# LLNL/Juqbox.jl

Hardware: AMD Instinct MI355X
Metric: traceobjgrad evals/sec (fwd+adjoint), cnot3 Hilbert dim (higher is better)
Workload: dtype f64

## Files before the change

### juqbox.jl_amd/csrc/jq_kernels.h

```cpp
#pragma once
#include <hip/hip_runtime.h>
#include <stdint.h>
#include <type_traits>

typedef double d4 __attribute__((ext_vector_type(4)));

#define JQ_WAVES 4
#define JQ_MAXNC 4
#define JQ_NTR 5
#define JQ_STATE_ARRAYS 4
#define JQ_STATE_EXTRA 8
#define JQ_MAXSLOTS 2
#define JQ_MAXSCHED 30

#define JQ_BW_OD 9
#define JQ_OD_COEFS(NT) (32 * (NT))

#define JQ_BW_T4 8
#define JQ_BW_T4Q 7
#define JQ_T4_AIDX(rho, k, i) (((rho) >> 2) * 64 + 16 * (k) + 4 * ((rho) & 3) + (i))
#define JQ_T4_TILE 16
#define JQ_T4_COEFS(NT) (64 * (NT))
#define JQ_T4_CIDX(g, r, t) ((g) * 16 + (r) * 4 + (t))
#define JQ_T4_CPOS(r, t) (4 * (r) + (t))
// ... 56 lines not shown
__device__ __forceinline__ s1 operator*(const s1& a, const s1& b) { return s1(a.e[0] * b.e[0]); }
__device__ __forceinline__ s1 operator*(double c, const s1& b) { return s1(c * b.e[0]); }
__device__ __forceinline__ s1 operator-(const s1& a) { return s1(-a.e[0]); }
__device__ __forceinline__ double row_sum(const d4& p) { return (p[0] + p[1]) + (p[2] + p[3]); }
__device__ __forceinline__ double row_sum(const s4& p) { return (p[0] + p[1]) + (p[2] + p[3]); }
__device__ __forceinline__ double row_sum(const s1& p) { return p[0]; }
#if defined(JQ_BW) && JQ_BW == 7
typedef s1 jq_row;
#define JQ_RL 1
#elif defined(JQ_BW) && JQ_BW == 8 && !defined(JQ_ROW_D4)
typedef s4 jq_row;
#define JQ_RL 4
#else
typedef d4 jq_row;
#define JQ_RL 4
#endif

template <int NT>
struct Arr {
    jq_row t[NT];
};

template <int NT>
__device__ __forceinline__ void a_zero(Arr<NT>& a)
{
#pragma unroll
    for (int i = 0; i < NT; ++i) a.t[i] = (d4){0.0, 0.0, 0.0, 0.0};
}
template <int NT>
__device__ __forceinline__ void a_axpy(Arr<NT>& y, double c, const Arr<NT>& x)
{
#pragma unroll
    for (int i = 0; i < NT; ++i) y.t[i] += c * x.t[i];
}
template <int NT>
__device__ __forceinline__ void a_add(Arr<NT>& y, const Arr<NT>& x)
{
#pragma unroll
    for (int i = 0; i < NT; ++i) y.t[i] += x.t[i];
}
template <int NT>
__device__ __forceinline__ void a_neg(Arr<NT>& y)
{
#pragma unroll
    for (int i = 0; i < NT; ++i) y.t[i] = -y.t[i];
}
template <int NT>
__device__ __forceinline__ double a_dot(const Arr<NT>& x, const Arr<NT>& y)
{
    double s = 0.0;
#pragma unroll
    for (int i = 0; i < NT; ++i) {
#if JQ_RL == 1 && defined(JQ_EXP_DOTFMA)
        s = fma(x.t[i][0], y.t[i][0], s);
#else
        s += row_sum(x.t[i] * y.t[i]);
#endif
    }
    return s;
}
template <int NT>
__device__ __forceinline__ void a_axpy_rows(Arr<NT>& y, double c, const double* tab, int g, const Arr<NT>& x)
{
#if JQ_RL == 1
#pragma unroll
    for (int i = 0; i < NT; ++i) y.t[i][0] = fma(c * tab[16 * i + g], x.t[i][0], y.t[i][0]);
#else
    const d4* t4 = (const d4*)(tab + 4 * g);
#pragma unroll
    for (int i = 0; i < NT; ++i) y.t[i] += jq_row(c * t4[4 * i]) * x.t[i];
#endif
}
template <int NT, bool NEG>
__device__ __forceinline__ void a_axpy_rows1(Arr<NT>& y, const double* tab, int g, const Arr<NT>& x)
{
#if JQ_RL == 1
#pragma unroll
    for (int i = 0; i < NT; ++i) y.t[i][0] = fma(NEG ? -tab[16 * i + g] : tab[16 * i + g], x.t[i][0], y.t[i][0]);
#else
    const d4* t4 = (const d4*)(tab + 4 * g);
#pragma unroll
    for (int i = 0; i < NT; ++i) y.t[i] += jq_row(NEG ? -t4[4 * i] : t4[4 * i]) * x.t[i];
#endif
}
template <int NT>
__device__ __forceinline__ double a_wsq(const double* tab, int g, const Arr<NT>& x)
{
    double s = 0.0;
#pragma unroll
    for (int i = 0; i < NT; ++i)
#pragma unroll
        for (int r = 0; r < JQ_RL; ++r) s += tab[16 * i + (JQ_RL == 1 ? g : 4 * g + r)] * (x.t[i][r] * x.t[i][r]);
    return s;
}

template <int NT>
__device__ __forceinline__ void a_load(Arr<NT>& a, const double* __restrict__ img, int lane)
{
#pragma unroll
    for (int i = 0; i < NT; ++i)
#pragma unroll
        for (int r = 0; r < JQ_RL; ++r) a.t[i][r] = img[(4 * i + r) * 64 + lane];
}
template <int NT>
__device__ __forceinline__ void a_store(const Arr<NT>& a, double* __restrict__ img, int lane)
{
#pragma unroll
    for (int i = 0; i < NT; ++i)
#pragma unroll
        for (int r = 0; r < JQ_RL; ++r) img[(4 * i + r) * 64 + lane] = a.t[i][r];
}

#define JQ_PF 4

template <int NT, bool ZEROC, bool SD>
__device__ __forceinline__ void mm_od(Arr<NT>& D, const Arr<NT>& C, const double* mat, const Arr<NT>& x)
{
    constexpr int NTILES = SD ? 0 : 4 * NT;
    const int lane = threadIdx.x & 63;
    const double* cf = mat - lane + NTILES * 64 + (lane >> 4) * 4;
    const d4 zero = {0.0, 0.0, 0.0, 0.0};
    d4 ca = *(const d4*)(cf), cb = *(const d4*)(cf + 16);
    if constexpr (SD) {
        d4 x_prev = zero, x_cur = x.t[0];
#pragma unroll
        for (int mt = 0; mt < NT; ++mt) {
            const d4 x_next = (mt + 1 < NT) ? x.t[mt + 1] : zero;
            d4 acc = ZEROC ? zero : C.t[mt];
            if (mt > 0) acc += ca * x_prev;
            if (mt + 1 < NT) acc += cb * x_next;
            if (mt + 1 < NT) {
                ca = *(const d4*)(cf + ((mt + 1) * 2 + 0) * 16);
                cb = *(const d4*)(cf + ((mt + 1) * 2 + 1) * 16);
            }
            D.t[mt] = acc;
            x_prev = x_cur;
            x_cur = x_next;
        }
        return;
    } else {
        double f[JQ_PF];
#pragma unroll
        for (int i = 0; i < JQ_PF; ++i)
            if (i < NTILES) f[i] = mat[i * 64];
        d4 x_cur = x.t[0];
        d4 nxt = ZEROC ? zero : C.t[0];
        if (NT > 1) nxt += cb * x.t[1];
        if (NT > 1) {
            ca = *(const d4*)(cf + 2 * 16);
            cb = *(const d4*)(cf + 3 * 16);
        }
#pragma unroll
        for (int mt = 0; mt < NT; ++mt) {
            const d4 x_next = (mt + 1 < NT) ? x.t[mt + 1] : zero;
            d4 acc = nxt;
#pragma unroll
            for (int k = 0; k < 4; ++k) {
                const int kk = 4 * mt + k;
                const double a = f[kk % JQ_PF];
                if (kk + JQ_PF < NTILES) f[kk % JQ_PF] = mat[(kk + JQ_PF) * 64];
                acc = __builtin_amdgcn_mfma_f64_16x16x4f64(a, x_cur[k], acc, 0, 0, 0);
                __builtin_amdgcn_sched_barrier(0);
                if (k == 0 && mt + 1 < NT) {
                    nxt = ZEROC ? zero : C.t[mt + 1];
                    nxt += ca * x_cur;
                    if (mt + 2 < NT) nxt += cb * x.t[mt + 2];
// ... 286 lines not shown
};
template <int NT, int NP, bool Z0, bool Z1, bool Z2, int SH = 0, typename HOOK = T4qNoHook, int SCM = 0>
__device__ __forceinline__ void mm_t4q_multi(Arr<NT>& D0, const Arr<NT>& C0, const double* m0, Arr<NT>& D1, const Arr<NT>& C1,
                                             const double* m1, Arr<NT>& D2, const Arr<NT>& C2, const double* m2, const Arr<NT>& x,
                                             double sh0 = 0.0, double sh1 = 0.0, double sh2 = 0.0, const double* wsr = nullptr,
                                             HOOK hook = HOOK())
{
    const int lane = threadIdx.x & 63;
    const double* ma[3] = {t4q_a(m0, lane), t4q_a(m1, lane), t4q_a(NP > 2 ? m2 : m1, lane)};
    const d4* cf[3] = {t4q_c<NT>(m0, lane), t4q_c<NT>(m1, lane), t4q_c<NT>(NP > 2 ? m2 : m1, lane)};
    double xold = 0.0;
    double as[3];
    d2 cs[3];
#pragma unroll
    for (int k = 0; k < NP; ++k)
        if ((SCM >> k) & 1) {
            as[k] = ma[k][0];
            cs[k] = t4s_c01(cf[k]);
        }
#pragma unroll
    for (int mt = 0; mt < NT; ++mt) {
        double a[3];
        d4 c[3];
#pragma unroll
        for (int k = 0; k < NP; ++k) {
            if ((SCM >> k) & 1) {
                a[k] = as[k];
                c[k] = t4s_c(cs[k], t4s_c23(cf[k], mt));
            } else {
                a[k] = ma[k][mt * 64];
                c[k] = t4q_cload(cf[k], mt);
            }
        }
        if constexpr (SH != 0) {
            const double w = wsr[16 * mt];
            if constexpr (SH & 1) a[0] = fma(sh0, w, a[0]);
            if constexpr (NP > 1 && (SH & 2)) a[1] = fma(sh1, w, a[1]);
            if constexpr (NP > 2 && (SH & 4)) a[2] = fma(sh2, w, a[2]);
        }
        const double xc = x.t[mt][0], xn = x.t[mt + 1 < NT ? mt + 1 : mt][0];
        const double su = row_shift4<0x114>(xc), sd = row_shift4<0x104>(xc);
        hook(mt, su, sd);
        double acc[3] = {Z0 ? 0.0 : C0.t[mt][0], (NP > 1 && !Z1) ? C1.t[mt][0] : 0.0, (NP > 2 && !Z2) ? C2.t[mt][0] : 0.0};
#ifndef JQ_EXP_MFMA_LAST
#pragma unroll
        for (int k = 0; k < NP; ++k) acc[k] = __builtin_amdgcn_mfma_f64_4x4x4f64(a[k], xc, acc[k], 0, 0, 0);
#endif
#pragma unroll
        for (int k = 0; k < NP; ++k) acc[k] = fma(c[k][0], su, acc[k]);
#pragma unroll
        for (int k = 0; k < NP; ++k) acc[k] = fma(c[k][1], sd, acc[k]);
        if (mt > 0) {
#pragma unroll
            for (int k = 0; k < NP; ++k) acc[k] = fma(c[k][2], xold, acc[k]);
        }
        if (mt + 1 < NT) {
#pragma unroll
            for (int k = 0; k < NP; ++k) acc[k] = fma(c[k][3], xn, acc[k]);
        }
#ifdef JQ_EXP_MFMA_LAST
#pragma unroll
        for (int k = 0; k < NP; ++k) acc[k] = __builtin_amdgcn_mfma_f64_4x4x4f64(a[k], xc, acc[k], 0, 0, 0);
#endif
        xold = xc;
        D0.t[mt][0] = acc[0];
        if constexpr (NP > 1) D1.t[mt][0] = acc[1];
        if constexpr (NP > 2) D2.t[mt][0] = acc[2];
        __builtin_amdgcn_sched_barrier(0);
    }
}
template <int NT, bool Z0, bool Z1, int SH = 0, int SCM = 0>
__device__ __forceinline__ void mm_t4q2(Arr<NT>& D0, const Arr<NT>& C0, const double* m0, Arr<NT>& D1, const Arr<NT>& C1,
                                        const double* m1, const Arr<NT>& x, double sh0 = 0.0, double sh1 = 0.0, const double* wsr = nullptr)
{
    mm_t4q_multi<NT, 2, Z0, Z1, true, SH, T4qNoHook, SCM>(D0, C0, m0, D1, C1, m1, D1, C1, m1, x, sh0, sh1, 0.0, wsr);
}
template <int NT, bool Z0, bool Z1, bool Z2, int SH = 0, int SCM = 0>
__device__ __forceinline__ void mm_t4q3(Arr<NT>& D0, const Arr<NT>& C0, const double* m0, Arr<NT>& D1, const Arr<NT>& C1,
                                        const double* m1, Arr<NT>& D2, const Arr<NT>& C2, const double* m2, const Arr<NT>& x,
                                        double sh0 = 0.0, double sh1 = 0.0, double sh2 = 0.0, const double* wsr = nullptr)
{
    mm_t4q_multi<NT, 3, Z0, Z1, Z2, SH, T4qNoHook, SCM>(D0, C0, m0, D1, C1, m1, D2, C2, m2, x, sh0, sh1, sh2, wsr);
}
template <int NT>
__device__ __forceinline__ void t4q_load(OpQ<NT>& op, const double* mat)
{
    const int lane = threadIdx.x & 63;
    const double* ma = t4q_a(mat, lane);
    const d4* cf = t4q_c<NT>(mat, lane);
#pragma unroll
    for (int mt = 0; mt < NT; ++mt) {
        op.a[mt] = ma[mt * 64];
#ifdef JQ_EXP_OPQ_EDGE
        const double* cd = (const double*)(cf + mt * 16);
        op.c[mt][0] = cd[0], op.c[mt][1] = cd[1];
        op.c[mt][2] = mt > 0 ? cd[2] : 0.0;
        op.c[mt][3] = mt + 1 < NT ? cd[3] : 0.0;
#else
        op.c[mt] = t4q_cload(cf, mt);
#endif
    }
}
template <int NT>
__device__ __forceinline__ void mm_t4q_regs(Arr<NT>& D, const Arr<NT>& C, const OpQ<NT>& op, const Arr<NT>& x)
{
    double xold = 0.0;
#pragma unroll
    for (int mt = 0; mt < NT; ++mt) t4q_block<NT, false, JQ_T4_DIAG | JQ_T4_RTERMS | JQ_T4_MTERMS>(D, C, x, mt, op.a[mt], op.c[mt], xold);
}

template <int NT>
struct OpS {
    double a;
    d2 c;
    d2 m[NT];
};
template <int NT>
__device__ __forceinline__ void t4s_load(OpS<NT>& op, const double* mat)
{
    const int lane = threadIdx.x & 63;
    const d4* cf = t4q_c<NT>(mat, lane);
    op.a = t4q_a(mat, lane)[0];
    op.c = t4s_c01(cf);
#pragma unroll
    for (int mt = 0; mt < NT; ++mt) op.m[mt] = t4s_c23(cf, mt);
}
template <int NT>
__device__ __forceinline__ void mm_t4s_regs(Arr<NT>& D, const Arr<NT>& C, const OpS<NT>& op, const Arr<NT>& x)
{
    double xold = 0.0;
#pragma unroll
    for (int mt = 0; mt < NT; ++mt)
        t4q_block<NT, false, JQ_T4_DIAG | JQ_T4_RTERMS | JQ_T4_MTERMS>(D, C, x, mt, op.a, t4s_c(op.c, op.m[mt]), xold);
}
template <int NT, bool ZEROC>
__device__ __forceinline__ void mm_t4s(Arr<NT>& D, const Arr<NT>& C, const double* mat, const Arr<NT>& x)
{
    const int lane = threadIdx.x & 63;
    const d4* cf = t4q_c<NT>(mat, lane);
    const double a = t4q_a(mat, lane)[0];
    const d2 c01 = t4s_c01(cf);
    d2 m_cur = t4s_c23(cf, 0);
    double xold = 0.0;
#pragma unroll
    for (int mt = 0; mt < NT; ++mt) {
        const d2 m = m_cur;
        if (mt + 1 < NT) m_cur = t4s_c23(cf, mt + 1);
        t4q_block<NT, ZEROC, JQ_T4_DIAG | JQ_T4_RTERMS | JQ_T4_MTERMS>(D, C, x, mt, a, t4s_c(c01, m), xold);
    }
}

template <int NT, int BW, bool ZEROC, bool SD = false>
__device__ __forceinline__ void mm_band(Arr<NT>& D, const Arr<NT>& C, const double* mat, const Arr<NT>& x);
template <int NT, int BW, bool ZEROC, bool SD = false>
__device__ __forceinline__ void mm_any(Arr<NT>& D, const Arr<NT>& C, const double* mat, const Arr<NT>& x)
{
    if constexpr (BW == JQ_BW_T4)
        mm_t4<NT, ZEROC, JQ_T4_DIAG | JQ_T4_RTERMS | JQ_T4_MTERMS>(D, C, mat, x);
    else if constexpr (BW == JQ_BW_T4Q)
        mm_t4q<NT, ZEROC, JQ_T4_DIAG | JQ_T4_RTERMS | JQ_T4_MTERMS>(D, C, mat, x);
    else if constexpr (BW == JQ_BW_OD)
        mm_od<NT, ZEROC, SD>(D, C, mat, x);
    else
        mm_band<NT, BW, ZEROC, SD>(D, C, mat, x);
}
template <int NT, int BW, bool ZEROC, bool SD>
// ... 54 lines not shown
        case JQ_T4_MTERMS: mm_t4q<NT, true, JQ_T4_MTERMS>(D, D, mat, x); break;
        default: mm_t4q<NT, true, JQ_T4_DIAG | JQ_T4_RTERMS | JQ_T4_MTERMS>(D, D, mat, x); break;
        }
    } else {
        if (BW > 0 && mode == 0)
            mm_any<NT, 0, true>(D, D, mat, x);
        else if (BW > 0 && NT > 1 && mode == 2)
            mm_any<NT, BW, true, true>(D, D, mat, x);
        else
            mm_any<NT, BW, true>(D, D, mat, x);
    }
}

template <int N>
__device__ __forceinline__ double row_ror_add(double x)
{
    union {
        double d;
        int i[2];
    } a, b;
    a.d = x;
    b.i[0] = __builtin_amdgcn_update_dpp(0, a.i[0], 0x120 + N, 0xf, 0xf, false);
    b.i[1] = __builtin_amdgcn_update_dpp(0, a.i[1], 0x120 + N, 0xf, 0xf, false);
    return x + b.d;
}
__device__ __forceinline__ double lane_bcast(double x, int l)
{
    union {
        double d;
        int i[2];
    } a, b;
    a.d = x;
    b.i[0] = __builtin_amdgcn_readlane(a.i[0], l);
    b.i[1] = __builtin_amdgcn_readlane(a.i[1], l);
    return b.d;
}
__device__ __forceinline__ double wave_sum(double x)
{
    x = row_ror_add<8>(x);
    x = row_ror_add<4>(x);
    x = row_ror_add<2>(x);
    x = row_ror_add<1>(x);
    return (lane_bcast(x, 0) + lane_bcast(x, 16)) + (lane_bcast(x, 32) + lane_bcast(x, 48));
}

__device__ __forceinline__ double wave_sum_hi(double x)
{
    x = row_ror_add<8>(x);
    x = row_ror_add<4>(x);
    x = row_ror_add<2>(x);
    x = row_ror_add<1>(x);
    union {
        double d;
        int i[2];
    } a, b;
    a.d = x;
    b.i[0] = __builtin_amdgcn_update_dpp(0, a.i[0], 0x142, 0xa, 0xf, false);
    b.i[1] = __builtin_amdgcn_update_dpp(0, a.i[1], 0x142, 0xa, 0xf, false);
    x += b.d;
    a.d = x;
    b.i[0] = __builtin_amdgcn_update_dpp(0, a.i[0], 0x143, 0xc, 0xf, false);
    b.i[1] = __builtin_amdgcn_update_dpp(0, a.i[1], 0x143, 0xc, 0xf, false);
    return x + b.d;
}

typedef unsigned jq_u2 __attribute__((ext_vector_type(2)));
__device__ __forceinline__ void row_swap32(double& a, double& b)
{
    union { double d; unsigned u[2]; } x, y;
    x.d = a, y.d = b;
    const jq_u2 lo = __builtin_amdgcn_permlane32_swap(x.u[0], y.u[0], false, false);
    const jq_u2 hi = __builtin_amdgcn_permlane32_swap(x.u[1], y.u[1], false, false);
    x.u[0] = lo[0], y.u[0] = lo[1], x.u[1] = hi[0], y.u[1] = hi[1];
    a = x.d, b = y.d;
}
__device__ __forceinline__ void row_swap16(double& a, double& b)
{
    union { double d; unsigned u[2]; } x, y;
    x.d = a, y.d = b;
    const jq_u2 lo = __builtin_amdgcn_permlane16_swap(x.u[0], y.u[0], false, false);
    const jq_u2 hi = __builtin_amdgcn_permlane16_swap(x.u[1], y.u[1], false, false);
    x.u[0] = lo[0], y.u[0] = lo[1], x.u[1] = hi[0], y.u[1] = hi[1];
    a = x.d, b = y.d;
}
__device__ __forceinline__ double wave_sum4(double a, double b, double c, double d)
{
    row_swap32(a, b);
    double p = a + b;
    row_swap32(c, d);
    double q = c + d;
    row_swap16(p, q);
    double r = p + q;
    r = row_ror_add<8>(r);
    r = row_ror_add<4>(r);
    r = row_ror_add<2>(r);
    return row_ror_add<1>(r);
}
__device__ __forceinline__ double wave_sum4_rows(double r0, double r1, double r2, double r3) { return wave_sum4(r0, r2, r1, r3); }
__device__ __forceinline__ double wave_sum2(double a, double b)
{
    row_swap32(a, b);
    double p = a + b;
    double q = p;
    row_swap16(p, q);
    double r = p + q;
    r = row_ror_add<8>(r);
    r = row_ror_add<4>(r);
    r = row_ror_add<2>(r);
    return row_ror_add<1>(r);
}
struct SchedEntry {
    int kind;
    int tp;
};

struct PropArgs {
    const double* stream;
    const double* cimg;
    double* state;
    const double* colinfo;
    double* traces;
    double* hist_r;
    double* hist_i;
    const double* tabs;
    double* park;
    long long stride;
    long long state_stride;
    int pieces;
    int nslots;
    int nsteps_chunk;
    int m;
    int nslabs;
    int Ncoupled;
    int step0;
    int first_chunk;
    int Ntot, N;
    int parts;
    int nsamples, sps;
    int qps;
    int use_shift;
    int forced;
    int debug;
    int park_lds;
    int batch;
    int lds_tab_off;
    int period;
    int npro;
    int bw_trace[JQ_MAXNC];
    double h;
    double tinv;
    double jacobi_tol2;
    unsigned long long sched_bits[3];
    unsigned long long pro_bits;
    const double* wlr;
    int wrank;
    int wstride;
    int wlr_lds;
    int wlr_sc_lds;
    int jac_wg_lds;
    int wcplx;
    int wlam;
    int rdv_polls;
    int wait_polls;
    long long stream_gstride;
};
__device__ __forceinline__ const double* jq_group_stream(const PropArgs& a, int unit, int upg)
// ... 517 lines not shown
    }
    mm_c<NT, BW>(Ya, A, S, A);
    --rem;
    if constexpr (BW == JQ_BW_OD || BW == JQ_BW_T4 || BW == JQ_BW_T4Q) {
        for (; rem > 0; --rem) mm_c<NT, BW>(Ya, A, S, Ya);
        mm_c<NT, BW>(out, bpa, S, Ya);
        return;
    }
    while (rem >= 2) {
        mm_c<NT, BW>(Yb, A, S, Ya);
        mm_c<NT, BW>(Ya, A, S, Yb);
        rem -= 2;
    }
    if (rem == 1) {
        mm_c<NT, BW>(Yb, A, S, Ya);
        mm_c<NT, BW>(out, bpa, S, Yb);
    } else {
        mm_c<NT, BW>(out, bpa, S, Ya);
    }
}

#ifndef JQ_BWD_TERMS
#define JQ_BWD_TERMS 1
#endif
constexpr bool jq_bwd_terms(int NT, int BW, bool JAC) { return JQ_BWD_TERMS && !JAC && NT >= 6 && BW != JQ_BW_OD && BW != JQ_BW_T4 && BW != JQ_BW_T4Q; }
template <int NT, int BW>
__device__ __forceinline__ void neumann_terms_add(Arr<NT>& out, Arr<NT>& A, const double* S, int m, Arr<NT>& Ya)
{
    for (int j = 0; j < m; j += 2) {
        mm_z<NT, BW>(Ya, S, A);
        a_add(out, Ya);
        if (j + 1 < m) {
            mm_z<NT, BW>(A, S, Ya);
            a_add(out, A);
        }
    }
}

template <int NT>
__device__ __forceinline__ void a_park(const Arr<NT>& a, __attribute__((address_space(3))) double* park)
{
#pragma unroll
    for (int i = 0; i < NT; ++i)
#pragma unroll
        for (int r = 0; r < JQ_RL; ++r) park[(JQ_RL * i + r) * 64] = a.t[i][r];
}
template <int NT>
__device__ __forceinline__ void a_unpark(Arr<NT>& a, const __attribute__((address_space(3))) double* park)
{
#pragma unroll
    for (int i = 0; i < NT; ++i)
#pragma unroll
        for (int r = 0; r < JQ_RL; ++r) a.t[i][r] = park[(JQ_RL * i + r) * 64];
}
template <int NT>
__device__ __forceinline__ void a_park(const Arr<NT>& a, double* park)
{
#pragma unroll
    for (int i = 0; i < NT; ++i)
#pragma unroll
        for (int r = 0; r < JQ_RL; ++r) park[(JQ_RL * i + r) * 64] = a.t[i][r];
}
template <int NT>
__device__ __forceinline__ void a_unpark(Arr<NT>& a, const double* park)
{
#pragma unroll
    for (int i = 0; i < NT; ++i)
#pragma unroll
        for (int r = 0; r < JQ_RL; ++r) a.t[i][r] = park[(JQ_RL * i + r) * 64];
}

#ifndef JQ_FWD_FUSE
#define JQ_FWD_FUSE 3
#endif
#ifndef JQ_BWD_FUSE
#define JQ_BWD_FUSE 3
#endif
#ifndef JQ_BWD_FUSE3
#define JQ_BWD_FUSE3 0
#endif
#ifndef JQ_BWD_ADJ_FUSE
#define JQ_BWD_ADJ_FUSE 1
#endif
#ifndef JQ_BWD3_NOOPQ
#define JQ_BWD3_NOOPQ 0
#endif
#ifndef JQ_BWD3_NOOPQ_STATE
#define JQ_BWD3_NOOPQ_STATE 0
#endif
template <int NT, int BW, bool JAC, int FUSE = 0, bool FOLD = false, bool REGOP = true, bool TERMS = false, typename RING = RingT<BW == JQ_BW_T4Q>, bool SC = false>
__device__ __forceinline__ void sv_state(RING& p, const PropArgs& a, bool active, double ceps, const double* ws, int g,
                                         const Arr<NT>& u, Arr<NT>& v, Arr<NT>& unew, Arr<NT>& vN, Arr<NT>& A, Arr<NT>& Ya,
                                         Arr<NT>& Yb)
{
    static_assert(!SC || (BW == JQ_BW_T4Q && !JAC && FUSE == 3 && REGOP), "SC: the fused quad-layout step");
    if constexpr (BW == JQ_BW_T4Q && !JAC && FUSE != 0) {
        const double* M0 = p.template next_ks<0, 1>();
        const double* M1 = p.template next_ks<1, 0>();
        if (active) {
            if constexpr (FOLD) {
                static_assert(!FOLD || (FUSE & 3) == 3 || FUSE == 0, "FOLD: fused or generic path");
                mm_t4q2<NT, true, false, 1, SC ? 2 : 0>(A, A, M0, unew, u, M1, u, ceps, 0.0, ws + g);
            } else {
            if constexpr (FUSE & 1) {
                mm_t4q2<NT, true, false, 0, SC ? 2 : 0>(A, A, M0, unew, u, M1, u);
            } else {
                mm_z<NT, BW>(A, M0, u);
                mm_c<NT, BW>(unew, u, M1, u);
            }
            if (a.use_shift) a_axpy_rows(A, ceps, ws, g, u);
            }
        }
        M0 = p.template next_ks<1, 1>();
        if (active) {
            if constexpr (SC) mm_t4s<NT, false>(A, A, M0, v);
            else mm_c<NT, BW>(A, A, M0, v);
            a_add(v, A);
            horner_add<NT, BW, JAC, REGOP, SC>(v, v, A, M0, a.m, Ya, Yb, a.jacobi_tol2, a.N, a.jac_wg_lds);
        }
        M1 = p.template next_ks<0, 0>();
        const double* M2 = p.template next_ks<0, 2>();
        if (active) {
            if constexpr (FOLD) {
                mm_t4q3<NT, false, false, true, 6, SC ? 1 : 0>(vN, v, M0, unew, unew, M1, A, A, M2, v, 0.0, -ceps, -ceps, ws + g);
            } else {
            if constexpr (FUSE & 2) {
                mm_t4q3<NT, false, false, true, 0, SC ? 1 : 0>(vN, v, M0, unew, unew, M1, A, A, M2, v);
            } else {
                mm_c<NT, BW>(vN, v, M0, v);
                mm_c<NT, BW>(unew, unew, M1, v);
                mm_z<NT, BW>(A, M2, v);
            }
            if (a.use_shift) {
                a_axpy_rows(unew, -ceps, ws, g, v);
                a_axpy_rows(A, -ceps, ws, g, v);
            }
            }
        }
        M0 = p.template next_ks<1, 2>();
        if (active) {
            if constexpr (SC) mm_t4s<NT, false>(A, A, M0, unew);
            else mm_c<NT, BW>(A, A, M0, unew);
            a_add(unew, A);
            horner_add<NT, BW, JAC, REGOP, SC>(unew, unew, A, M0, a.m, Ya, Yb, a.jacobi_tol2, a.N, a.jac_wg_lds);
        }
        return;
    }
    constexpr int FULLQ = JQ_T4_DIAG | JQ_T4_RTERMS | JQ_T4_MTERMS;
    const double* M = p.template next_ks<0, 1>();
    if (active) {
        if constexpr (FOLD) {
            mm_t4q<NT, true, FULLQ, true>(A, A, M, u, ceps, ws + g);
        } else {
            mm_z<NT, BW>(A, M, u);
            if (a.use_shift) a_axpy_rows(A, ceps, ws, g, u);
        }
    }
    M = p.template next_ks<1, 1>();
    if (active) {
        mm_c<NT, BW>(A, A, M, v);
        a_add(v, A);
        if constexpr (TERMS) neumann_terms_add<NT, BW>(v, A, M, a.m, Ya);
        else horner_add<NT, BW, JAC, REGOP>(v, v, A, M, a.m, Ya, Yb, a.jacobi_tol2, a.N, a.jac_wg_lds);
        mm_c<NT, BW>(vN, v, M, v);
    }
    M = p.template next_ks<0, 0>();
    if (active) {
        if constexpr (FOLD) {
            mm_t4q<NT, false, FULLQ, true>(unew, u, M, v, -ceps, ws + g);
        } else {
            mm_c<NT, BW>(unew, u, M, v);
            if (a.use_shift) a_axpy_rows(unew, -ceps, ws, g, v);
        }
    }
    M = p.template next_ks<1, 0>();
    if (active) mm_c<NT, BW>(unew, unew, M, u);
    M = p.template next_ks<0, 2>();
    if (active) {
        if constexpr (FOLD) {
            mm_t4q<NT, true, FULLQ, true>(A, A, M, v, -ceps, ws + g);
        } else {
            mm_z<NT, BW>(A, M, v);
            if (a.use_shift) a_axpy_rows(A, -ceps, ws, g, v);
        }
    }
    M = p.template next_ks<1, 2>();
    if (active) {
        mm_c<NT, BW>(A, A, M, unew);
        a_add(unew, A);
        if constexpr (TERMS) neumann_terms_add<NT, BW>(unew, A, M, a.m, Ya);
        else horner_add<NT, BW, JAC, REGOP>(unew, unew, A, M, a.m, Ya, Yb, a.jacobi_tol2, a.N, a.jac_wg_lds);
    }
}

template <int BW, bool JAC, bool WLRT>
constexpr bool jq_wlr_on() { return WLRT; }
template <int NT, int BW, int MINW, bool JAC, bool WLRT = false, bool UNI = false, bool SC = false>
__global__ __launch_bounds__((BW == JQ_BW_T4Q) ? 256 * MINW : 256, (BW == JQ_BW_T4Q) ? 1 : MINW) void k_forward(PropArgs a)
{
    static_assert(!SC || (BW == JQ_BW_T4Q && MINW == 3 && !JAC && !WLRT), "SC: a variant of the three-slab quad-layout kernel");
    extern __shared__ __attribute__((aligned(16))) char smem[];
    constexpr int KT = 4 * NT;
    const int lane_ = threadIdx.x & 63;
    const int wave = __builtin_amdgcn_readfirstlane(threadIdx.x >> 6);
    constexpr bool QUAD = (BW == JQ_BW_T4Q);
    constexpr int NWAVES = QUAD ? JQ_WAVES * MINW : JQ_WAVES;
    const int col = QUAD ? 4 * (wave & 3) + (lane_ & 3) : (lane_ & 15);
    const int lane = QUAD ? ((lane_ >> 2) & 3) * 64 + 16 * (lane_ >> 4) + col : lane_;
    const int g = QUAD ? 4 * (lane_ >> 4) + ((lane_ >> 2) & 3) : lane_ >> 4;
    const int wpw = (JAC && !QUAD) ? (int)(blockDim.x >> 6) : JQ_WAVES;
    const int slab = QUAD ? (int)blockIdx.x * (NWAVES / 4) + (wave >> 2) : blockIdx.x * wpw + wave;
    const bool active = slab < a.nslabs;

    double* tab = (double*)(smem + a.lds_tab_off);
    const double* wd = tab;
    const double* ws = tab + 16 * NT;
    for (int i = threadIdx.x; i < 32 * NT; i += blockDim.x) tab[(i & ~15) + 4 * (i & 3) + ((i >> 2) & 3)] = a.tabs[i];

    Arr<NT> ua, va, ub, vb, A, Ya, Yb;
    double leak = 0.0, ceps = 0.0;
    double* st = a.state + (size_t)(active ? slab : 0) * a.state_stride;
    if (active) {
        a_load(ua, st, lane);
        a_load(va, st + KT * 64, lane);
        leak = (!QUAD || ((lane_ >> 2) & 3) == 0) ? st[(JQ_STATE_ARRAYS * KT + JQ_MAXNC) * 64 + (QUAD ? 16 * (lane_ >> 4) + col : lane)] : 0.0;
        ceps = 0.5 * a.h * a.colinfo[(size_t)slab * 32 + col];
        if constexpr (UNI) ceps = (a.use_shift && (lane_ >> 4) == (lane_ & 3)) ? lane_bcast(ceps, 0) : 0.0;
    } else {
        a_zero(ua);
        a_zero(va);
    }
    RingT<QUAD> p;
    p.init(smem, a, wave, lane_, QUAD ? NWAVES : wpw);
    constexpr bool WLR = jq_wlr_on<BW, JAC, WLRT>();
    WLow<NT, QUAD> wl;
    if constexpr (WLR) wl.init(a, lane_, smem);

#define JQ_FWD_STEP(U, V, UN, VN, NSTEP)                                                                         \
    {                                                                                                            \
        p.begin_step(NSTEP);                                                                                     \
        if (active) leak += a_wsq(wd, g, U);                   \
        sv_state<NT, BW, JAC, JQ_FWD_FUSE, UNI, true, false, RingT<QUAD>, SC>(p, a, active, ceps, ws, g, U, V, UN, VN, A, Ya, Yb); \
                                                \
        const double* M6 = p.template next_ks<0, 1>();                                                                             \
        if (active) {                                                                                            \
            if constexpr (UNI) {                                                                                 \
                mm_t4q<NT, false, JQ_T4_DIAG | JQ_T4_RTERMS | JQ_T4_MTERMS, true>(VN, VN, M6, UN, ceps, ws + g);   \
            } else {                                                                                             \
                mm_c<NT, BW>(VN, VN, M6, UN);                                                                    \
                if (a.use_shift) a_axpy_rows(VN, ceps, ws, g, UN);                                               \
            }                                                                                                    \
                   \
            leak += a_wsq(wd, g, UN) + 2.0 * a_wsq(wd, g, V);                                                    \
            if constexpr (WLR)                                                                                   \
                if (wl.r > 0) {    \
                    double lk = 0.0;                                                                             \
                    for (int k = 0; k < wl.r; ++k) {                                                             \
                        double p0, q0, p1, q1, rr, ss;                                                           \
                        if (wl.has_sc) p0 = wl.get(k, 0), q0 = wl.get(k, 1);       \
                        else wl.dots(k, U, p0, q0);                                                              \
                        wl.dots(k, UN, p1, q1);                                                                  \
                        if (wl.has_sc) wl.put(k, 0, p1), wl.put(k, 1, q1);                                       \
                        wl.dots(k, V, rr, ss);                                                                   \
                        lk += wl.lam(k) * ((p0 * p0 + q0 * q0) + (p1 * p1 + q1 * q1) + 2.0 * (rr * rr + ss * ss) - 2.0 * (ss * p0 - rr * q0)); \
                    }                                                                                            \
                    if (wl.lead) leak += lk;                                                                     \
                }                                                                                                \
            if (a.hist_r) hist_store<NT>(a, slab, col, QUAD ? 4 * ((lane_ >> 2) & 3) + (lane_ >> 4) : g, NSTEP, UN, VN); \
        }                                                                                                        \
    }
    if constexpr (WLR)
        if (wl.has_sc && active)
            for (int k = 0; k < wl.r; ++k) {
                double p0, q0;
                wl.dots(k, ua, p0, q0);
                wl.put(k, 0, p0), wl.put(k, 1, q0);
            }
    int n = 0;
    for (; n + 1 < a.nsteps_chunk; n += 2) {
        JQ_FWD_STEP(ua, va, ub, vb, n)
        JQ_FWD_STEP(ub, vb, ua, va, n + 1)
    }
    if (n < a.nsteps_chunk) {
        JQ_FWD_STEP(ua, va, ub, vb, n)
        if (active) {
            ua = ub;
            va = vb;
        }
    }
#undef JQ_FWD_STEP
    p.drain();
    if (active) {
        a_store(ua, st, lane);
        a_store(va, st + KT * 64, lane);
        if constexpr (QUAD) {
            leak = row_ror_add<8>(row_ror_add<4>(leak));
            if (((lane_ >> 2) & 3) == 0) st[(JQ_STATE_ARRAYS * KT + JQ_MAXNC) * 64 + 16 * (lane_ >> 4) + col] = leak;
        } else {
            st[(JQ_STATE_ARRAYS * KT + JQ_MAXNC) * 64 + lane] = leak;
        }
    }
}

template <int NT, int BW, int MINW, bool JAC, bool WLRT = false, bool UNI = false, bool ORD = false, bool SC = false>
__global__ __launch_bounds__((BW == JQ_BW_T4Q) ? 256 * MINW : 256, (BW == JQ_BW_T4Q) ? 1 : MINW) void k_backward(PropArgs a)
{
    static_assert(!ORD || (UNI && BW == JQ_BW_T4Q && !JAC), "ORD: a variant of the UNI quad-layout kernel");
    static_assert(!SC || (ORD && MINW == 3 && !WLRT && !JQ_BWD3_NOOPQ && !JQ_BWD3_NOOPQ_STATE), "SC: a variant of the ORD three-slab kernel");
    extern __shared__ __attribute__((aligned(16))) char smem[];
    constexpr int KT = 4 * NT;
    const int lane_ = threadIdx.x & 63;
    const int wave = __builtin_amdgcn_readfirstlane(threadIdx.x >> 6);
    constexpr bool QUAD = (BW == JQ_BW_T4Q);
    constexpr int NWAVES = QUAD ? JQ_WAVES * MINW : JQ_WAVES;
    constexpr int NTHREADS = 64 * NWAVES;
    const int col = QUAD ? 4 * (wave & 3) + (lane_ & 3) : (lane_ & 15);
    const int lane = QUAD ? ((lane_ >> 2) & 3) * 64 + 16 * (lane_ >> 4) + col : lane_;
    const int g = QUAD ? 4 * (lane_ >> 4) + ((lane_ >> 2) & 3) : lane_ >> 4;
    const int wpw = (JAC && !QUAD) ? (int)(blockDim.x >> 6) : JQ_WAVES;
    const int slab = QUAD ? (int)blockIdx.x * (NWAVES / 4) + (wave >> 2) : blockIdx.x * wpw + wave;
    const bool active = slab < a.nslabs;
    const int Nc = a.Ncoupled;
    const bool cslot = !QUAD || ((lane_ >> 2) & 3) == 0;
    const int clane = QUAD ? 16 * (lane_ >> 4) + col : lane_;

    double* tab = (double*)(smem + a.lds_tab_off);
    const double* wd = tab;
    const double* ws = tab + 16 * NT;
    double* carry = tab + 32 * NT;
    const double cfw = a.forced ? 0.5 * a.h * a.tinv : 0.0;
    for (int i = threadIdx.x; i < 32 * NT; i += blockDim.x)
        tab[(i & ~15) + 4 * (i & 3) + ((i >> 2) & 3)] = (i < 16 * NT) ? cfw * a.tabs[i] : a.tabs[i];
    double* st = a.state + (size_t)(active ? slab : 0) * a.state_stride;
    typedef __attribute__((address_space(3))) double lds_double;
    typedef typename std::conditional<QUAD, lds_double*, double*>::type park_ptr;
    park_ptr P0;
    if constexpr (QUAD)
        P0 = (lds_double*)(carry + Nc * NTHREADS + (size_t)wave * (JQ_RL * NT) * 64 + lane_);
    else
        P0 = a.park_lds ? (carry + Nc * NTHREADS + (size_t)wave * (JQ_RL * NT) * 64 + lane_)
                        : (a.park + (size_t)(active ? slab : 0) * KT * 64 + lane);
    const int ntr = Nc * JQ_NTR;
    double* rec = carry + Nc * NTHREADS + (a.park_lds ? (size_t)NWAVES * (JQ_RL * NT) * 64 : 0);
    const int rslots = 8 * Nc;
    for (int i = threadIdx.x; i < 2 * NWAVES * rslots; i += blockDim.x) rec[i] = 0.0;
    auto flush_traces = [&](int k) {
        if (!QUAD && a.batch > 0) {
            asm volatile("s_waitcnt lgkmcnt(0)" ::: "memory");
            __builtin_amdgcn_s_barrier();
            asm volatile("" ::: "memory");
        }
        if (wave == 0 && lane_ < ntr) {
            const int q = lane_ / JQ_NTR, kk = lane_ - q * JQ_NTR;
            const int slot = (kk == 0 ? 0 : kk == 2 ? 2 : 4 * Nc + (kk == 1 ? 0 : kk == 3 ? 2 : 1)) + 4 * q;
            const double* r = rec + (size_t)(k & 1) * NWAVES * rslots + slot;
            double s = r[0];
#pragma unroll
            for (int w = 1; w < NWAVES; ++w) s += r[w * rslots];
            a.traces[((size_t)blockIdx.x * a.nsteps_chunk + k) * ntr + lane_] = s;
        }
    };

    Arr<NT> u, v, mu, nb, un, vN, L, Ya, Yb;
    double ceps = 0.0, wgt = 0.0;
    if (active) {
        a_load(u, st, lane);
        a_load(v, st + KT * 64, lane);
        a_load(mu, st + 2 * KT * 64, lane);
        a_load(nb, st + 3 * KT * 64, lane);
        ceps = 0.5 * a.h * a.colinfo[(size_t)slab * 32 + col];
        wgt = a.colinfo[(size_t)slab * 32 + 16 + col];
        if constexpr (UNI) {
            wgt = lane_bcast(wgt, 0);
            ceps = (a.use_shift && (lane_ >> 4) == (lane_ & 3)) ? lane_bcast(ceps, 0) : 0.0;
        }
        for (int q = 0; q < Nc; ++q) carry[q * NTHREADS + threadIdx.x] = cslot ? st[(JQ_STATE_ARRAYS * KT + q) * 64 + clane] : 0.0;
    } else {
        a_zero(u);
        a_zero(v);
        a_zero(mu);
        a_zero(nb);
    }
    RingT<QUAD> p;
    p.init(smem, a, wave, lane_, QUAD ? NWAVES : wpw);
    constexpr bool WLR = jq_wlr_on<BW, JAC, WLRT>();
    WLow<NT, QUAD> wl;
    if constexpr (WLR) wl.init(a, lane_, smem);
    const bool wforce = WLR && a.wrank > 0 && a.forced;
    constexpr bool BREG = !(QUAD && MINW >= 3 && JQ_BWD3_NOOPQ);

    if (a.first_chunk) {
        for (int q = 0; q < Nc; ++q) {
            const double* M = p.next_c(q);
            if (active) {
                mm_z_bw<NT, BW>(Ya, M, nb, a.bw_trace[q]);
                carry[q * NTHREADS + threadIdx.x] = -a_dot(u, Ya);
            }
        }
    }

    if constexpr (WLR)
        if (wforce && wl.has_sc && active)
            for (int k = 0; k < wl.r; ++k) {
                double pu, qu;
                wl.dots(k, u, pu, qu);
                wl.put(k, 0, pu), wl.put(k, 1, qu);
            }
    for (int n = 0; n < a.nsteps_chunk; ++n) {
        p.begin_step(n);
        if (active) a_park(mu, P0);
        sv_state<NT, BW, JAC, (MINW >= 3 ? (UNI ? 3 : JQ_BWD_FUSE3) : JQ_BWD_FUSE), UNI, !(QUAD && MINW >= 3 && JQ_BWD3_NOOPQ_STATE), jq_bwd_terms(NT, BW, JAC), RingT<QUAD>, SC>(p, a, active, ceps, ws, g, u, v, un, vN, mu, Ya, Yb);
        if (n > 0) flush_traces(n - 1);
        const double* M = p.template next_ks<0, 1>();
        if (active) {
            if constexpr (UNI) {
                constexpr int FULLQ = JQ_T4_DIAG | JQ_T4_RTERMS | JQ_T4_MTERMS;
                mm_t4q<NT, false, FULLQ, true>(vN, vN, M, un, ceps, ws + g);
                mm_t4q<NT, true, FULLQ, true>(L, L, M, nb, ceps, ws + g);
            } else {
                mm_c<NT, BW>(vN, vN, M, un);
                if (a.use_shift) a_axpy_rows(vN, ceps, ws, g, un);
                mm_z<NT, BW>(L, M, nb);
                if (a.use_shift) a_axpy_rows(L, ceps, ws, g, nb);
            }
            a_unpark(mu, P0);
            a_park(vN, P0);
        }
        M = p.template next_ks<1, 0>();
        if (active) {
            if constexpr (SC) mm_t4s<NT, false>(L, L, M, mu);
            else mm_c<NT, BW>(L, L, M, mu);
            a_axpy_rows1<NT, false>(L, wd, g, u);
            if constexpr (WLR)
                if (wforce)
                    for (int k = 0; k < wl.r; ++k) {
                        double pu, qu;
                        if (wl.has_sc) pu = wl.get(k, 0), qu = wl.get(k, 1);
                        else wl.dots(k, u, pu, qu);
                        const double cl = cfw * wl.lam(k);
                        wl.axpy2(k, L, cl * pu, cl * qu);
                    }
            a_add(mu, L);
            if constexpr (jq_bwd_terms(NT, BW, JAC)) neumann_terms_add<NT, BW>(mu, L, M, a.m, Ya);
            else horner_add<NT, BW, JAC, BREG, SC>(mu, mu, L, M, a.m, Ya, Yb, a.jacobi_tol2, a.N, a.jac_wg_lds);
        }
        double o_p4 = 0.0;
        for (int q = 0; q < Nc; ++q) {
            M = p.next_c(Nc + q);
            if (active) {
                if constexpr (ORD) {
                    if (q == 0) mm_t4q<NT, true, JQ_T4_DIAG>(Ya, Ya, M, mu);
                    else if (q == 1) mm_t4q<NT, true, JQ_T4_RTERMS>(Ya, Ya, M, mu);
                    else mm_t4q<NT, true, JQ_T4_MTERMS>(Ya, Ya, M, mu);
                } else {
                    mm_z_bw<NT, BW>(Ya, M, mu, a.bw_trace[q]);
                }
                const double ts = UNI ? wave_sum4(a_dot(u, Ya), a_dot(un, Ya), 0.0, 0.0) * wgt
                                      : wave_sum4(a_dot(u, Ya) * wgt, a_dot(un, Ya) * wgt, 0.0, 0.0);
                if ((lane_ & 15) == 0) rec[((size_t)(n & 1) * NWAVES + wave) * rslots + 4 * q + (lane_ >> 4)] = ts;
            }
        }
        if constexpr (QUAD && !JAC && (JQ_BWD_ADJ_FUSE & 1)) {
            M = p.template next_ks<0, 0>();
            const double* M9 = p.template next_ks<0, 2>();
            if (active) {
                if constexpr (UNI) {
                    mm_t4q2<NT, true, true, 3>(L, L, M, vN, vN, M9, mu, -ceps, -ceps, ws + g);
                } else {
                    mm_t4q2<NT, true, true>(L, L, M, vN, vN, M9, mu);
                    if (a.use_shift) {
                        a_axpy_rows(L, -ceps, ws, g, mu);
                        a_axpy_rows(vN, -ceps, ws, g, mu);
                    }
                }
            }
        } else {
        M = p.template next_ks<0, 0>();
        if (active) {
            mm_z<NT, BW>(L, M, mu);
            if (a.use_shift) a_axpy_rows(L, -ceps, ws, g, mu);
        }
        M = p.template next_ks<0, 2>();
        if (active) {
            mm_z<NT, BW>(vN, M, mu);
            if (a.use_shift) a_axpy_rows(vN, -ceps, ws, g, mu);
        }
        }
        M = p.template next_ks<1, 1>();
        if (active) {
            if constexpr (SC) mm_t4s<NT, true>(Ya, Ya, M, nb);
            else mm_z<NT, BW>(Ya, M, nb);
            a_axpy_rows1<NT, true>(Ya, wd, g, v);
            if constexpr (WLR)
                if (wforce)
                    for (int k = 0; k < wl.r; ++k) {
                        double pn, qn, rr, ss;
                        wl.dots(k, un, pn, qn);
                        wl.dots(k, v, rr, ss);
                        if (wl.has_sc) wl.put(k, 2, pn), wl.put(k, 3, qn), wl.put(k, 4, rr), wl.put(k, 5, ss);
                        const double cl = cfw * wl.lam(k);
                        wl.axpy2(k, Ya, -cl * rr, -cl * ss);
                        wl.axpy2(k, vN, -cl * qn, cl * pn);
                    }
            a_add(L, Ya);
            a_add(vN, Ya);
            if constexpr (SC) mm_t4s<NT, false>(vN, vN, M, L);
            else mm_c<NT, BW>(vN, vN, M, L);
            a_add(L, nb);
            a_add(L, vN);
            if constexpr (jq_bwd_terms(NT, BW, JAC)) neumann_terms_add<NT, BW>(L, vN, M, a.m, Ya);
            else horner_add<NT, BW, JAC, BREG, SC>(L, L, vN, M, a.m, Ya, Yb, a.jacobi_tol2, a.N, a.jac_wg_lds);
            a_add(nb, L);
        }
        M = p.template next_ks<0, 1>();
        if (active) {
            if constexpr (ORD) {
                const d4* cfs = t4q_c<NT>(p.next_c(1), lane_);
                mm_t4q_multi<NT, 1, false, true, true, 1>(vN, mu, M, vN, mu, M, vN, mu, M, L, ceps, 0.0, 0.0, ws + g,
                                                          [&](int mt, double su, double sd) {
                                                              const d4 cs = t4q_cload(cfs, mt);
                                                              o_p4 = fma(-un.t[mt][0], fma(cs[1], sd, cs[0] * su), o_p4);
                                                          });
            } else if constexpr (UNI) {
                mm_t4q<NT, false, JQ_T4_DIAG | JQ_T4_RTERMS | JQ_T4_MTERMS, true>(vN, mu, M, L, ceps, ws + g);
            } else {
                mm_c<NT, BW>(vN, mu, M, L);
                if (a.use_shift) a_axpy_rows(vN, ceps, ws, g, L);
            }
        }
        M = p.template next_ks<1, 2>();
        if (active) {
            if constexpr (SC) mm_t4s<NT, false>(vN, vN, M, mu);
            else mm_c<NT, BW>(vN, vN, M, mu);
            a_axpy_rows1<NT, false>(vN, wd, g, un);
            if constexpr (WLR)
                if (wforce)
                    for (int k = 0; k < wl.r; ++k) {
                        double pn, qn, rr, ss;
                        if (wl.has_sc) {
                            pn = wl.get(k, 2), qn = wl.get(k, 3), rr = wl.get(k, 4), ss = wl.get(k, 5);
                            wl.put(k, 0, pn), wl.put(k, 1, qn);
                        } else {
                            wl.dots(k, un, pn, qn);
                            wl.dots(k, v, rr, ss);
                        }
                        const double cl = cfw * wl.lam(k);
                        wl.axpy2(k, vN, cl * (pn - ss), cl * (qn + rr));
                    }
        }
        for (int q = 0; q < Nc; ++q) {
            double t2 = 0, t4 = 0, t5 = 0;
            const int bwq = a.bw_trace[q];
            M = p.next_c(Nc + q);
            if (active) {
                if constexpr (ORD) {
                    if (q == 0) mm_t4q<NT, true, JQ_T4_DIAG>(Ya, Ya, M, nb);
                    else if (q == 1) mm_t4q<NT, true, JQ_T4_RTERMS>(Ya, Ya, M, nb);
                    else mm_t4q<NT, true, JQ_T4_MTERMS>(Ya, Ya, M, nb);
                } else {
                    mm_z_bw<NT, BW>(Ya, M, nb, bwq);
                }
                t5 = -a_dot(v, Ya);
            }
            M = p.next_c(q);
            if (active) {
                double p4;
                if constexpr (ORD) {
                    if (q == 1) {
                        mm_t4q<NT, true, JQ_T4_RTERMS>(Ya, Ya, M, mu);
                        t2 = a_dot(v, Ya);
                        p4 = o_p4;
                    } else {
                        if (q == 0) mm_t4q<NT, true, JQ_T4_DIAG>(Ya, Ya, M, mu);
                        else mm_t4q<NT, true, JQ_T4_MTERMS>(Ya, Ya, M, mu);
                        t2 = a_dot(v, Ya);
                        if (q == 0) mm_t4q<NT, true, JQ_T4_DIAG>(Ya, Ya, M, L);
                        else mm_t4q<NT, true, JQ_T4_MTERMS>(Ya, Ya, M, L);
                        p4 = -a_dot(un, Ya);
                    }
                } else {
                    mm_z_bw<NT, BW>(Ya, M, mu, bwq);
                    t2 = a_dot(v, Ya);
                    mm_z_bw<NT, BW>(Ya, M, L, bwq);
                    p4 = -a_dot(un, Ya);
                }
                t4 = p4 + carry[q * NTHREADS + threadIdx.x];
                carry[q * NTHREADS + threadIdx.x] = p4;
                const double ts = UNI ? wave_sum4(t2, t4, t5, 0.0) * wgt : wave_sum4(t2 * wgt, t4 * wgt, t5 * wgt, 0.0);
                if ((lane_ & 15) == 0) rec[((size_t)(n & 1) * NWAVES + wave) * rslots + 4 * (Nc + q) + (lane_ >> 4)] = ts;
            }
        }
        if (active) {
            u = un;
            mu = vN;
            nb = L;
            a_unpark(v, P0);
        }
    }
    p.drain();
    flush_traces(a.nsteps_chunk - 1);
    if (active) {
        a_store(u, st, lane);
        a_store(v, st + KT * 64, lane);
        a_store(mu, st + 2 * KT * 64, lane);
        a_store(nb, st + 3 * KT * 64, lane);
        for (int q = 0; q < Nc; ++q) {
            double cv = carry[q * NTHREADS + threadIdx.x];
            if constexpr (QUAD) cv = row_ror_add<8>(row_ror_add<4>(cv));
            if (cslot) st[(JQ_STATE_ARRAYS * KT + q) * 64 + clane] = cv;
        }
    }
}
```

Before: 3057.

## Trim per-step work in fused quad-layout forward and adjoint steps

```diff
diff --git a/juqbox.jl_amd/csrc/jq_kernels.h b/juqbox.jl_amd/csrc/jq_kernels.h
--- a/juqbox.jl_amd/csrc/jq_kernels.h
+++ b/juqbox.jl_amd/csrc/jq_kernels.h
@@ -162,6 +162,12 @@
 #pragma unroll
     for (int i = 0; i < NT; ++i) y.t[i] += jq_row(NEG ? -t4[4 * i] : t4[4 * i]) * x.t[i];
 #endif
+}
+template <int NT, bool NEG>
+__device__ __forceinline__ void a_axpy_cw(Arr<NT>& y, const double* cw, const Arr<NT>& x)
+{
+#pragma unroll
+    for (int i = 0; i < NT; ++i) y.t[i][0] = fma(NEG ? -cw[i] : cw[i], x.t[i][0], y.t[i][0]);
 }
 template <int NT>
 __device__ __forceinline__ double a_wsq(const double* tab, int g, const Arr<NT>& x)
@@ -614,6 +620,40 @@
 {
     mm_t4q_multi<NT, 3, Z0, Z1, Z2, SH, T4qNoHook, SCM>(D0, C0, m0, D1, C1, m1, D2, C2, m2, x, sh0, sh1, sh2, wsr);
 }
+template <int NT, bool Z0, bool Z1>
+__device__ __forceinline__ void mm_t4q_2rhs(Arr<NT>& D0, const Arr<NT>& C0, const Arr<NT>& x0, Arr<NT>& D1, const Arr<NT>& C1,
+                                            const Arr<NT>& x1, const double* mat, double shd, const double* wsr)
+{
+    const int lane = threadIdx.x & 63;
+    const double* ma = t4q_a(mat, lane);
+    const d4* cf = t4q_c<NT>(mat, lane);
+    double xold0 = 0.0, xold1 = 0.0;
+#pragma unroll
+    for (int mt = 0; mt < NT; ++mt) {
+        const double a = fma(shd, wsr[16 * mt], ma[mt * 64]);
+        const d4 c = t4q_cload(cf, mt);
+        const double xc0 = x0.t[mt][0], xc1 = x1.t[mt][0];
+        double acc0 = Z0 ? 0.0 : C0.t[mt][0], acc1 = Z1 ? 0.0 : C1.t[mt][0];
+        acc0 = __builtin_amdgcn_mfma_f64_4x4x4f64(a, xc0, acc0, 0, 0, 0);
+        acc1 = __builtin_amdgcn_mfma_f64_4x4x4f64(a, xc1, acc1, 0, 0, 0);
+        acc0 = fma(c[0], row_shift4<0x114>(xc0), acc0);
+        acc1 = fma(c[0], row_shift4<0x114>(xc1), acc1);
+        acc0 = fma(c[1], row_shift4<0x104>(xc0), acc0);
+        acc1 = fma(c[1], row_shift4<0x104>(xc1), acc1);
+        if (mt > 0) {
+            acc0 = fma(c[2], xold0, acc0);
+            acc1 = fma(c[2], xold1, acc1);
+        }
+        if (mt + 1 < NT) {
+            acc0 = fma(c[3], x0.t[mt + 1 < NT ? mt + 1 : mt][0], acc0);
+            acc1 = fma(c[3], x1.t[mt + 1 < NT ? mt + 1 : mt][0], acc1);
+        }
+        xold0 = xc0, xold1 = xc1;
+        D0.t[mt][0] = acc0;
+        D1.t[mt][0] = acc1;
+        __builtin_amdgcn_sched_barrier(0);
+    }
+}
 template <int NT>
 __device__ __forceinline__ void t4q_load(OpQ<NT>& op, const double* mat)
 {
@@ -834,6 +874,20 @@
     const jq_u2 hi = __builtin_amdgcn_permlane16_swap(x.u[1], y.u[1], false, false);
     x.u[0] = lo[0], y.u[0] = lo[1], x.u[1] = hi[0], y.u[1] = hi[1];
     a = x.d, b = y.d;
+}
+__device__ __forceinline__ double wave_sum4_half(double a, double b)
+{
+    row_swap32(a, b);
+    return a + b;
+}
+__device__ __forceinline__ double wave_sum4_join(double p, double q)
+{
+    row_swap16(p, q);
+    double r = p + q;
+    r = row_ror_add<8>(r);
+    r = row_ror_add<4>(r);
+    r = row_ror_add<2>(r);
+    return row_ror_add<1>(r);
 }
 __device__ __forceinline__ double wave_sum4(double a, double b, double c, double d)
 {
@@ -1517,17 +1571,21 @@
 #ifndef JQ_BWD_ADJ_FUSE
 #define JQ_BWD_ADJ_FUSE 1
 #endif
+#ifndef JQ_STEP_TRIM
+#define JQ_STEP_TRIM 7
+#endif
 #ifndef JQ_BWD3_NOOPQ
 #define JQ_BWD3_NOOPQ 0
 #endif
 #ifndef JQ_BWD3_NOOPQ_STATE
 #define JQ_BWD3_NOOPQ_STATE 0
 #endif
-template <int NT, int BW, bool JAC, int FUSE = 0, bool FOLD = false, bool REGOP = true, bool TERMS = false, typename RING = RingT<BW == JQ_BW_T4Q>, bool SC = false>
+template <int NT, int BW, bool JAC, int FUSE = 0, bool FOLD = false, bool REGOP = true, bool TERMS = false, typename RING = RingT<BW == JQ_BW_T4Q>, bool SC = false, bool CW = false>
 __device__ __forceinline__ void sv_state(RING& p, const PropArgs& a, bool active, double ceps, const double* ws, int g,
                                          const Arr<NT>& u, Arr<NT>& v, Arr<NT>& unew, Arr<NT>& vN, Arr<NT>& A, Arr<NT>& Ya,
-                                         Arr<NT>& Yb)
-{
+                                         Arr<NT>& Yb, const double* cw = nullptr)
+{
+    static_assert(!CW || (BW == JQ_BW_T4Q && !JAC && FUSE != 0 && !FOLD), "CW: the fused quad-layout step with the shift applied to the results");
     static_assert(!SC || (BW == JQ_BW_T4Q && !JAC && FUSE == 3 && REGOP), "SC: the fused quad-layout step");
     if constexpr (BW == JQ_BW_T4Q && !JAC && FUSE != 0) {
         const double* M0 = p.template next_ks<0, 1>();
@@ -1543,7 +1601,10 @@
                 mm_z<NT, BW>(A, M0, u);
                 mm_c<NT, BW>(unew, u, M1, u);
             }
-            if (a.use_shift) a_axpy_rows(A, ceps, ws, g, u);
+            if (a.use_shift) {
+                if constexpr (CW) a_axpy_cw<NT, false>(A, cw, u);
+                else a_axpy_rows(A, ceps, ws, g, u);
+            }
             }
         }
         M0 = p.template next_ks<1, 1>();
@@ -1567,8 +1628,13 @@
                 mm_z<NT, BW>(A, M2, v);
             }
             if (a.use_shift) {
-                a_axpy_rows(unew, -ceps, ws, g, v);
-                a_axpy_rows(A, -ceps, ws, g, v);
+                if constexpr (CW) {
+                    a_axpy_cw<NT, true>(unew, cw, v);
+                    a_axpy_cw<NT, true>(A, cw, v);
+                } else {
+                    a_axpy_rows(unew, -ceps, ws, g, v);
+                    a_axpy_rows(A, -ceps, ws, g, v);
+                }
             }
             }
         }
@@ -1671,11 +1737,15 @@
     WLow<NT, QUAD> wl;
     if constexpr (WLR) wl.init(a, lane_, smem);
 
+    constexpr bool TRIM3 = QUAD && MINW == 3 && !JAC && !UNI && JQ_FWD_FUSE != 0;
+    constexpr bool LKC = TRIM3 && (JQ_STEP_TRIM & 1), CWH = TRIM3 && (JQ_STEP_TRIM & 2);
+    double lw = 0.0;
+    double cw[CWH ? NT : 1] = {};
 #define JQ_FWD_STEP(U, V, UN, VN, NSTEP)                                                                         \
     {                                                                                                            \
         p.begin_step(NSTEP);                                                                                     \
-        if (active) leak += a_wsq(wd, g, U);                   \
-        sv_state<NT, BW, JAC, JQ_FWD_FUSE, UNI, true, false, RingT<QUAD>, SC>(p, a, active, ceps, ws, g, U, V, UN, VN, A, Ya, Yb); \
+        if (active) leak += LKC ? lw : a_wsq(wd, g, U);        \
+        sv_state<NT, BW, JAC, JQ_FWD_FUSE, UNI, true, false, RingT<QUAD>, SC, CWH>(p, a, active, ceps, ws, g, U, V, UN, VN, A, Ya, Yb, cw); \
                                                 \
         const double* M6 = p.template next_ks<0, 1>();                                                                             \
         if (active) {                                                                                            \
@@ -1683,10 +1753,14 @@
                 mm_t4q<NT, false, JQ_T4_DIAG | JQ_T4_RTERMS | JQ_T4_MTERMS, true>(VN, VN, M6, UN, ceps, ws + g);   \
             } else {                                                                                             \
                 mm_c<NT, BW>(VN, VN, M6, UN);                                                                    \
-                if (a.use_shift) a_axpy_rows(VN, ceps, ws, g, UN);                                               \
+                if (a.use_shift) {                                                                               \
+                    if constexpr (CWH) a_axpy_cw<NT, false>(VN, cw, UN);                                         \
+                    else a_axpy_rows(VN, ceps, ws, g, UN);                                                       \
+                }                                                                                                \
             }                                                                                                    \
                    \
-            leak += a_wsq(wd, g, UN) + 2.0 * a_wsq(wd, g, V);                                                    \
+            lw = a_wsq(wd, g, UN);                                                                               \
+            leak += lw + 2.0 * a_wsq(wd, g, V);                                                                  \
             if constexpr (WLR)                                                                                   \
                 if (wl.r > 0) {    \
                     double lk = 0.0;                                                                             \
@@ -1711,6 +1785,13 @@
                 wl.dots(k, ua, p0, q0);
                 wl.put(k, 0, p0), wl.put(k, 1, q0);
             }
+    if (active) {
+        if constexpr (LKC) lw = a_wsq(wd, g, ua);
+        if constexpr (CWH) {
+#pragma unroll
+            for (int i = 0; i < NT; ++i) cw[i] = ceps * ws[16 * i + g];
+        }
+    }
     int n = 0;
     for (; n + 1 < a.nsteps_chunk; n += 2) {
         JQ_FWD_STEP(ua, va, ub, vb, n)
@@ -1777,6 +1858,7 @@
                         : (a.park + (size_t)(active ? slab : 0) * KT * 64 + lane);
     const int ntr = Nc * JQ_NTR;
     double* rec = carry + Nc * NTHREADS + (a.park_lds ? (size_t)NWAVES * (JQ_RL * NT) * 64 : 0);
+    constexpr bool PK = ORD && MINW == 3 && (JQ_STEP_TRIM & 4);
     const int rslots = 8 * Nc;
     for (int i = threadIdx.x; i < 2 * NWAVES * rslots; i += blockDim.x) rec[i] = 0.0;
     auto flush_traces = [&](int k) {
@@ -1787,7 +1869,8 @@
         }
         if (wave == 0 && lane_ < ntr) {
             const int q = lane_ / JQ_NTR, kk = lane_ - q * JQ_NTR;
-            const int slot = (kk == 0 ? 0 : kk == 2 ? 2 : 4 * Nc + (kk == 1 ? 0 : kk == 3 ? 2 : 1)) + 4 * q;
+            const int slot = PK ? ((kk == 0 || kk == 2) ? (q == 1 ? 1 : 4 * (q >> 1)) + kk : 4 * ((Nc + 1) >> 1) + 4 * q + (kk == 1 ? 0 : kk == 3 ? 1 : 2))
+                                : (kk == 0 ? 0 : kk == 2 ? 2 : 4 * Nc + (kk == 1 ? 0 : kk == 3 ? 2 : 1)) + 4 * q;
             const double* r = rec + (size_t)(k & 1) * NWAVES * rslots + slot;
             double s = r[0];
 #pragma unroll
@@ -1850,8 +1933,12 @@
         if (active) {
             if constexpr (UNI) {
                 constexpr int FULLQ = JQ_T4_DIAG | JQ_T4_RTERMS | JQ_T4_MTERMS;
-                mm_t4q<NT, false, FULLQ, true>(vN, vN, M, un, ceps, ws + g);
-                mm_t4q<NT, true, FULLQ, true>(L, L, M, nb, ceps, ws + g);
+                if constexpr (MINW == 3 && (JQ_STEP_TRIM & 8)) {
+                    mm_t4q_2rhs<NT, false, true>(vN, vN, un, L, L, nb, M, ceps, ws + g);
+                } else {
+                    mm_t4q<NT, false, FULLQ, true>(vN, vN, M, un, ceps, ws + g);
+                    mm_t4q<NT, true, FULLQ, true>(L, L, M, nb, ceps, ws + g);
+                }
             } else {
                 mm_c<NT, BW>(vN, vN, M, un);
                 if (a.use_shift) a_axpy_rows(vN, ceps, ws, g, un);
@@ -1880,6 +1967,7 @@
             else horner_add<NT, BW, JAC, BREG, SC>(mu, mu, L, M, a.m, Ya, Yb, a.jacobi_tol2, a.N, a.jac_wg_lds);
         }
         double o_p4 = 0.0;
+        double pk = 0.0;
         for (int q = 0; q < Nc; ++q) {
             M = p.next_c(Nc + q);
             if (active) {
@@ -1889,6 +1977,19 @@
                     else mm_t4q<NT, true, JQ_T4_MTERMS>(Ya, Ya, M, mu);
                 } else {
                     mm_z_bw<NT, BW>(Ya, M, mu, a.bw_trace[q]);
+                }
+                if constexpr (PK) {
+                    const double d1 = a_dot(u, Ya), d3 = a_dot(un, Ya);
+                    const double hp = wave_sum4_half(d1, d3);
+                    if (q == 0) {
+                        pk = hp;
+                    } else {
+                        const double ts = (q == 1 ? wave_sum4_join(pk, hp) : wave_sum4_join(hp, wave_sum4_half(0.0, 0.0))) * wgt;
+                        int row = lane_ >> 4;
+                        asm volatile("" : "+v"(row));
+                        if ((lane_ & 15) == 0) rec[((size_t)(n & 1) * NWAVES + wave) * rslots + 4 * (q - 1) + row] = ts;
+                    }
+                    continue;
                 }
                 const double ts = UNI ? wave_sum4(a_dot(u, Ya), a_dot(un, Ya), 0.0, 0.0) * wgt
                                       : wave_sum4(a_dot(u, Ya) * wgt, a_dot(un, Ya) * wgt, 0.0, 0.0);
@@ -2021,6 +2122,13 @@
                 }
                 t4 = p4 + carry[q * NTHREADS + threadIdx.x];
                 carry[q * NTHREADS + threadIdx.x] = p4;
+                if constexpr (PK) {
+                    const double ts = wave_sum4_rows(t2, t4, t5, 0.0) * wgt;
+                    int row = lane_ >> 4;
+                    asm volatile("" : "+v"(row));
+                    if ((lane_ & 15) == 0) rec[((size_t)(n & 1) * NWAVES + wave) * rslots + 4 * (((Nc + 1) >> 1) + q) + row] = ts;
+                    continue;
+                }
                 const double ts = UNI ? wave_sum4(t2, t4, t5, 0.0) * wgt : wave_sum4(t2 * wgt, t4 * wgt, t5 * wgt, 0.0);
                 if ((lane_ & 15) == 0) rec[((size_t)(n & 1) * NWAVES + wave) * rslots + 4 * (Nc + q) + (lane_ >> 4)] = ts;
             }
@@ -2035,10 +2143,16 @@
     p.drain();
     flush_traces(a.nsteps_chunk - 1);
     if (active) {
-        a_store(u, st, lane);
-        a_store(v, st + KT * 64, lane);
-        a_store(mu, st + 2 * KT * 64, lane);
-        a_store(nb, st + 3 * KT * 64, lane);
+        int lane_s = lane;
+        if constexpr (PK) {
+            int l = lane_;
+            asm volatile("" : "+v"(l));
+            lane_s = ((l >> 2) & 3) * 64 + 16 * (l >> 4) + 4 * (wave & 3) + (l & 3);
+        }
+        a_store(u, st, lane_s);
+        a_store(v, st + KT * 64, lane_s);
+        a_store(mu, st + 2 * KT * 64, lane_s);
+        a_store(nb, st + 3 * KT * 64, lane_s);
         for (int q = 0; q < Nc; ++q) {
             double cv = carry[q * NTHREADS + threadIdx.x];
             if constexpr (QUAD) cv = row_ror_add<8>(row_ror_add<4>(cv));
```

New measurement: 3122, median of 6. 2.1% higher.
